# AnnSeidel/genometools

Hardware: AMD Instinct MI355X
Metric: Gbp/s ESA build (suf+lcp+bwt), 3 Gbp DNA, 1/2/4/8 MI355X; bit-exact vs CPU (higher is better)
Workload: dtype u64; 1 GPU; human-like DNA (2% N, 24 seqs, repeats) n=3000000000 seed=43 -suf -lcp -bwt (BASELINE.json configs[2]); parallelism=1 device, pair_suffixes=341032298, tied_suffixes=390540711, refine_rounds=9, maxbranchdepth=8256

## Files before the change

genometools_amd/_lib.py:

```python
import ctypes
import os
import subprocess

HERE = os.path.dirname(os.path.abspath(__file__))
ROOT = os.path.dirname(HERE)
LIB_PATH = os.path.join(HERE, "libgtamd_esa.so")
SOURCES = [os.path.join(HERE, "csrc", f) for f in
           ("esa_prims.hip", "esa_engine.hip", "esa_synth.hip", "esa_encode.hip",
            "esa_pck.hip", "esa_comm.hip")]
HEADERS = [os.path.join(HERE, "csrc", f) for f in ("esa_common.h", "esa_prims.h", "esa_devutil.h", "esa_msd.h", "esa_msd_blocks.h",
                                                     "esa_pck_replay.h")] + \
          [os.path.join(ROOT, "include", h) for h in ("gtamd_esa.h", "gtamd_encode.h", "gtamd_pck.h")]
HIPCC = os.environ.get("HIPCC", "/opt/rocm/bin/hipcc")


def needs_build():
    if not os.path.exists(LIB_PATH):
        return True
    t = os.path.getmtime(LIB_PATH)
    return any(os.path.getmtime(p) > t for p in SOURCES + HEADERS)


def build_library(force=False, verbose=False):
    if not force and not needs_build():
        return LIB_PATH
    cmd = [HIPCC, "--offload-arch=gfx950", "-O3", "-std=c++17", "-fPIC",
           "-shared", "-Wall", "-Wno-unused-function", "-o", LIB_PATH] + SOURCES
    if verbose:
        print(" ".join(cmd))
    subprocess.run(cmd, check=True)
    return LIB_PATH


class EsaStats(ctypes.Structure):
    _fields_ = [("totallength", ctypes.c_uint64),
                ("numberofallsortedsuffixes", ctypes.c_uint64),
                ("longest", ctypes.c_uint64),
                ("largelcpvalues", ctypes.c_uint64),
                ("maxbranchdepth", ctypes.c_uint64),
                ("lcptabsum", ctypes.c_uint64),
                ("prefixlength", ctypes.c_uint32),
                ("refine_rounds", ctypes.c_uint32),
                ("tied_suffixes", ctypes.c_uint64),
                ("pair_suffixes", ctypes.c_uint64),
                ("device_bytes", ctypes.c_uint64),
                ("msd_big_entries", ctypes.c_uint64),
                ("msd_crowded_entries", ctypes.c_uint64),
                ("rank_entries_built", ctypes.c_uint64)]


class EsaTiming(ctypes.Structure):
    _fields_ = [("total_ms", ctypes.c_float),
                ("keygen_ms", ctypes.c_float),
                ("sort_ms", ctypes.c_float),
                ("finalize_ms", ctypes.c_float),
                ("refine_ms", ctypes.c_float),
                ("tie_fix_ms", ctypes.c_float),
                ("scatter_ms", ctypes.c_float),
                ("scatter_launches", ctypes.c_uint32),
                ("scatter_items", ctypes.c_uint64),
                ("comm_ms", ctypes.c_float),
                ("comm_calls", ctypes.c_uint32),
                ("comm_bytes", ctypes.c_uint64),
                ("alloc_ms", ctypes.c_float),
                ("dominant_kernel", ctypes.c_uint32),
                ("scatter_read_items", ctypes.c_uint64),
                ("scatter_written_items", ctypes.c_uint64)]


class EncodeSummary(ctypes.Structure):
    _fields_ = [(name, ctypes.c_uint64) for name in
                ("totallength", "numofsequences", "specialcharacters",
                 "realspecialranges")] + \
               [("specialrangestab", ctypes.c_uint64 * 3)] + \
               [(name, ctypes.c_uint64) for name in
                ("lengthofspecialprefix", "lengthofspecialsuffix", "wildcards",
                 "realwildcardranges")] + \
               [("wildcardrangestab", ctypes.c_uint64 * 3)] + \
               [(name, ctypes.c_uint64) for name in
                ("lengthofwildcardprefix", "lengthofwildcardsuffix",
                 "lengthoflongestnonspecial", "minseqlen", "maxseqlen",
# ... 127 lines not shown
```

genometools_amd/csrc/esa_engine.hip:

```cpp
#include <stdarg.h>
#include <stdlib.h>
#include <chrono>
#include <type_traits>
#include <utility>
#include <vector>
#include "../../include/gtamd_esa.h"
#include "esa_prims.h"
#include "esa_devutil.h"

static thread_local char g_err[1024] = "";
void gtamd_set_error(const char *fmt, ...) {
  va_list ap;
  va_start(ap, fmt);
  vsnprintf(g_err, sizeof g_err, fmt, ap);
  va_end(ap);
}
extern "C" const char *gtamd_esa_last_error(void) { return g_err; }

extern "C" int gtamd_device_count(void) {
  GTAMD_ABI_BEGIN
  int n = 0;
  if (hipGetDeviceCount(&n) != hipSuccess) return 0;
  return n;
  GTAMD_ABI_END(0)
// ... 890 lines not shown
  }
  if (inbucket && (dc != 0 || longk)) {
    u32 letters = K::letters(key);
    if (dc == 0) {
      const u64 sp = sp_window(t, p + K::SYMS);
      letters += sp ? (u32) __ffsll((unsigned long long) sp) - 1u : 64u;
    }
    if (letters < k) {
      atomicAdd(&countspecial[bck_code_long<BITS>(t, key, p, k - 1, sigma)], 1u);
      if (letters >= 1 && letters + 2 <= k) {
        u64 off = 0, pw = sigma;
        for (u32 l = 1; l < letters; l++) { off += pw; pw *= sigma; }
        atomicAdd(&distpfx[off + bck_code_long<BITS>(t, key, p, letters, sigma)], 1u);
      }
    }
  }
}

struct Stats {
  unsigned long long numties;
  unsigned long long lcpsum;
  unsigned long long numlarge;
  unsigned long long longest;
  u32 maxlcp;
  u32 count;
  u32 count2;
  u32 dmax;
  unsigned long long dsum;
  u32 dfallback;
  u32 count3;
  unsigned long long smalldone;
  unsigned long long crowded;
  unsigned long long msum;
};

constexpr int FIN_THREADS = 256;
constexpr int FIN_PER_THREAD = 4;
constexpr int FIN_TILE = FIN_THREADS * FIN_PER_THREAD * 4;

template <int BITS>
__global__ __launch_bounds__(256) void k_tiebits(const u64 *__restrict__ keys,
                                                 u64 N, u64 *__restrict__ tiebits,
                                                 Stats *stats) {
  using K = Key<BITS>;
  __shared__ u32 s_cnt[4];
  const int lane = threadIdx.x & 63, w = threadIdx.x >> 6;
  u32 cnt = 0;
  const u64 ntiles = (N + 4095) / 4096;
  for (u64 tile = blockIdx.x; tile < ntiles; tile += gridDim.x) {
  const u64 wbase = tile * 4096 + (u64) w * 1024;
  u64 k[16];
#pragma unroll
  for (int r = 0; r < 16; r++) {
    const u64 i = wbase + (u64) r * 64 + lane;
    k[r] = i < N ? keys[i] : ~0ull;
  }
  u64 before = (wbase > 0 && wbase < N) ? keys[wbase - 1] : ~k[0];
#pragma unroll
  for (int r = 0; r < 16; r++) {
    const u64 i = wbase + (u64) r * 64 + lane;
    u64 prev = __shfl_up(k[r], 1, 64);
    if (lane == 0) prev = before;
    before = __shfl(k[r], 63, 64);
    const bool tie = i > 0 && i < N && (k[r] >> K::DSHIFT) == (prev >> K::DSHIFT) &&
                     K::dcode(k[r]) == 0;
    const u64 m = __ballot(tie);
// ... 834 lines not shown
      lcp[i + 1] = (u8) (lv < GTAMD_LCPOVERFLOW ? lv : GTAMD_LCPOVERFLOW);
      if (lv >= GTAMD_LCPOVERFLOW) lcpfull[i + 1] = lv;
    }
    if (r & PAIR_SWAP) {
      const u64 x = sa[i], y = sa[i + 1];
      if (x == 0) stats->longest = index_offset + i + 1;
      if (suf != nullptr) { suf[i] = y; suf[i + 1] = x; }
      if (bwt != nullptr) {
        const u8 b0 = bwt[i], b1 = bwt[i + 1];
        bwt[i] = b1;
        bwt[i + 1] = b0;
      }
    }
  }
}

constexpr int RT_TILE = 2048;
constexpr int RT_THREADS = 256;
constexpr int RT_PER = RT_TILE / RT_THREADS;

template <typename P> struct RoundKey {
  static constexpr int KK = sizeof(P) == 8 ? 40 : 32;
  static __device__ __forceinline__ u64 pack(u32 lg, bool open, u64 kk, u32 e) {
    return ((u64) lg << (12 + KK)) | ((u64) open << (11 + KK)) | (kk << 11) | (u64) e;
  }
  static __device__ __forceinline__ bool open(u64 key) { return (key >> (11 + KK)) & 1ull; }
};

template <typename P>
__global__ __launch_bounds__(RT_THREADS) void k_round_tile(
    const u32 *__restrict__ uidx, const P *__restrict__ upos,
    const u32 *__restrict__ ugrp, P *__restrict__ k2, u64 m,
    P *__restrict__ cv, u32 *__restrict__ hv, const u32 *__restrict__ tstart,
    u32 *__restrict__ flagbits, const P *__restrict__ rank, u64 h, u64 n) {
  using RK = RoundKey<P>;
  constexpr bool WIDE = sizeof(P) == 8;
  __shared__ u64 s_key[RT_TILE];
  __shared__ P s_pos[RT_TILE];
  __shared__ u64 s_k2w[WIDE ? RT_TILE : 1];
  __shared__ u16 s_start[RT_TILE + 2];
  __shared__ u32 s_scan[4];
  u32 *s_grp = reinterpret_cast<u32 *>(s_key);
  u32 *s_k2n = s_grp + RT_TILE;
  const int tid = threadIdx.x;
  const u64 tile_first = tstart[blockIdx.x], tile_end = tstart[blockIdx.x + 1];
  for (u64 base = tile_first; base < tile_end; base += RT_TILE) {
  const u32 cnt = (u32) ((tile_end - base) < (u64) RT_TILE ? (tile_end - base) : (u64) RT_TILE);
  const u32 g_first = ugrp[base], g_last = ugrp[base + cnt - 1];
  const bool first_open = base > 0 && ugrp[base - 1] == g_first;
  const bool last_open = base + cnt < m && ugrp[base + cnt] == g_last;
#pragma unroll
  for (int c = 0; c < RT_PER; c++) {
    const u32 e = (u32) c * RT_THREADS + tid;
    P kv = 0;
    if (e < cnt) {
      const P p = upos[base + e];
      s_grp[e] = ugrp[base + e];
      s_pos[e] = p;
      if (rank != nullptr) {
        u64 q = (u64) p + h;
        if (q > n) q = n;
        kv = rank[q];
      } else
        kv = k2[base + e];
    } else {
      s_grp[e] = 0xFFFFFFFFu;
      s_pos[e] = 0;
// ... 11 lines not shown
    gr[c] = s_grp[e0 + c];
    kr[c] = WIDE ? s_k2w[e0 + c] : (u64) s_k2n[e0 + c];
  }
  u32 startflags = 0, nstart = 0;
#pragma unroll
  for (int c = 0; c < RT_PER; c++) {
    const u32 e = e0 + c;
    const bool st = e == 0 || gr[c] != gprev;
    gprev = gr[c];
    startflags |= (u32) st << c;
    nstart += st;
  }
  u32 tot;
  u32 lg = block_scan_excl_sum(nstart, &tot, s_scan);
  u32 nflag = 0;
  int splits = 0;
  u32 openbits = 0;
#pragma unroll
  for (int c = 0; c < RT_PER; c++) {
    const u32 e = e0 + c;
    const bool start = (startflags >> c) & 1u;
    lg += start;
    const u32 g = gr[c];
    const bool open = e < cnt && ((first_open && g == g_first) ||
                                  (last_open && g == g_last));
    const u64 kraw = kr[c];
    const u64 kk = open ? 0ull : kraw;
    splits |= (e < cnt && !open && !start && kraw != kprev);
    kprev = kraw;
    s_key[e] = RK::pack(lg, open, kk, e);
    openbits |= (u32) open << c;
    if (open && rank != nullptr) k2[base + e] = (P) kraw;
    nflag += open;
  }
  if (openbits) {
#pragma unroll
    for (int c = 0; c < RT_PER; c++)
      if ((openbits >> c) & 1u) {
        const u64 slot = base + e0 + c;
        atomicOr(&flagbits[slot >> 5], 1u << (slot & 31));
      }
  }
  const int any_split = __syncthreads_or(splits);
  if (any_split) {
    {
      u32 lgw = lg;
#pragma unroll
      for (int c = RT_PER - 1; c >= 0; c--) {
        const u32 e = e0 + c;
        if ((startflags >> c) & 1u) { s_start[lgw] = (u16) e; lgw--; }
      }
      if (tid == 0) s_start[tot + 1] = (u16) RT_TILE;
    }
    __syncthreads();
    u32 gmax = 0;
    {
      u32 lgw = lg;
#pragma unroll
      for (int c = RT_PER - 1; c >= 0; c--) {
        const u32 e = e0 + c;
        if ((startflags >> c) & 1u) {
          const bool open = RK::open(s_key[e]);
          if (e < cnt && !open) {
            const u32 size = (u32) s_start[lgw + 1] - e;
            gmax = size > gmax ? size : gmax;
          }
// ... 35 lines not shown
            const bool up = (lo & k) == 0;
            const u64 a = s_key[lo], b = s_key[hi];
            if ((a > b) == up) { s_key[lo] = b; s_key[hi] = a; }
          }
          __syncthreads();
        }
      }
    }
  }
  u32 hval[RT_PER], hmax = 0;
#pragma unroll
  for (int c = 0; c < RT_PER; c++) {
    const u32 e = e0 + c;
    const u64 key = s_key[e];
    const bool head = e == 0 || (key >> 11) != (s_key[e - 1] >> 11);
    const u32 v = (head && e < cnt) ? uidx[base + e] : 0u;
    hval[c] = v;
    hmax = v > hmax ? v : hmax;
  }
  u32 carry = block_scan_excl_max(hmax, &tot, s_scan);
#pragma unroll
  for (int c = 0; c < RT_PER; c++) {
    const u32 e = e0 + c;
    carry = hval[c] > carry ? hval[c] : carry;
    if (e < cnt) {
      const u64 key = s_key[e];
      const u32 src = (u32) (key & 2047u);
      if (!RK::open(key)) {
        cv[base + e] = s_pos[src];
        hv[base + e] = carry;
      }
    }
  }
  (void) nflag;
  __syncthreads();
  }
}

constexpr int RT_STRIDE_MIN = 512;
__global__ __launch_bounds__(256) void k_tile_starts(const u32 *__restrict__ ugrp, u64 m,
                                                     u32 ntiles, u32 stride,
                                                     u32 *__restrict__ tstart) {
  const u32 t = blockIdx.x * 256 + threadIdx.x;
  if (t > ntiles) return;
  if (t == ntiles) { tstart[t] = (u32) m; return; }
  const u64 s = (u64) t * stride;
  const u32 g = ugrp[s];
  u64 lo = s > (u64) RT_TILE ? s - RT_TILE : 0, hi = s;
  if (ugrp[lo] == g) {
    tstart[t] = (u32) (lo == 0 ? 0 : s);
    return;
  }
  while (hi - lo > 1) {
    const u64 mid = (lo + hi) >> 1;
    if (ugrp[mid] == g) hi = mid; else lo = mid;
  }
  tstart[t] = (u32) hi;
}

__global__ __launch_bounds__(256) void k_flag_count(const u32 *__restrict__ flagbits, u64 m,
                                                    u32 nblocks, u32 *__restrict__ blkcnt) {
  const u32 b = blockIdx.x * 256 + threadIdx.x;
  if (b >= nblocks) return;
  u32 c = 0;
  for (int w = 0; w < RT_TILE / 32; w++) c += (u32) __popc(flagbits[(u64) b * (RT_TILE / 32) + w]);
  blkcnt[b] = c;
  (void) m;
}

template <typename P>
__global__ __launch_bounds__(RT_THREADS) void k_flag_gather(
    const u32 *__restrict__ flagbits, const u32 *__restrict__ tileoff,
    const u32 *__restrict__ ugrp, const P *__restrict__ k2,
    const P *__restrict__ upos, u64 m, P *__restrict__ fk2, P *__restrict__ fk2_sort,
    u32 *__restrict__ fgrp, P *__restrict__ fpos, u32 *__restrict__ fj,
    u32 *__restrict__ perm) {
  __shared__ u32 s_scan[4];
  const u64 base = (u64) blockIdx.x * RT_TILE + (u64) threadIdx.x * RT_PER;
// ... 21 lines not shown
                                                    const u32 *__restrict__ idx, u64 n,
                                                    u32 *__restrict__ dst) {
  const u64 r = (u64) blockIdx.x * 256 + threadIdx.x;
  if (r < n) dst[r] = src[idx[r]];
}

template <typename P>
__global__ __launch_bounds__(256) void k_flag_heads(
    const u32 *__restrict__ perm, const u32 *__restrict__ fgrp, const P *__restrict__ fk2,
    const P *__restrict__ fpos, const u32 *__restrict__ uidx, const u32 *__restrict__ fj,
    u64 nf, u32 *__restrict__ fhv, P *__restrict__ cvs) {
  const u64 r = (u64) blockIdx.x * 256 + threadIdx.x;
  if (r >= nf) return;
  const u32 a = perm[r];
  bool head = r == 0;
  if (!head) {
    const u32 b = perm[r - 1];
    head = fgrp[a] != fgrp[b] || fk2[a] != fk2[b];
  }
  fhv[r] = head ? uidx[fj[r]] : 0u;
  cvs[r] = fpos[a];
}

template <typename P>
__global__ __launch_bounds__(256) void k_flag_scatter(
    const P *__restrict__ cvs, const u32 *__restrict__ fhv,
    const u32 *__restrict__ fj, u64 nf, P *__restrict__ cv,
    u32 *__restrict__ hv) {
  const u64 r = (u64) blockIdx.x * 256 + threadIdx.x;
  if (r >= nf) return;
  const u32 j = fj[r];
  cv[j] = cvs[r];
  hv[j] = fhv[r];
}

template <typename P>
__global__ __launch_bounds__(256) void k_round_apply(
    const P *__restrict__ cval, const u32 *__restrict__ gnew,
    const u32 *__restrict__ uidx, const u32 *__restrict__ ugrp, u64 m,
    u64 rank_offset, P *__restrict__ sa, P *__restrict__ rank,
    u64 *__restrict__ keep, u32 *__restrict__ blockcnt) {
  __shared__ u32 s_cnt[4];
  const u64 j = (u64) blockIdx.x * 256 + threadIdx.x;
  bool kept = false;
  if (j < m) {
    const P p = cval[j];
    const u32 g = gnew[j], i = uidx[j];
    if (rank != nullptr && g != ugrp[j]) rank[p] = (P) (rank_offset + g);
    const bool head = g == i;
    const bool nexthead = j + 1 == m || gnew[j + 1] == uidx[j + 1];
    const bool resolved = head && nexthead;
    if (resolved) sa[i] = p;
    kept = !resolved;
  }
  const u64 b = __ballot(kept);
  if ((threadIdx.x & 63) == 0) {
    keep[((u64) blockIdx.x * 256 + threadIdx.x) >> 6] = b;
    s_cnt[threadIdx.x >> 6] = (u32) __popcll(b);
  }
  __syncthreads();
  if (threadIdx.x == 0) blockcnt[blockIdx.x] = s_cnt[0] + s_cnt[1] + s_cnt[2] + s_cnt[3];
}

template <typename P>
__global__ __launch_bounds__(256) void k_round_compact(
    const u64 *__restrict__ keep, const u32 *__restrict__ boff,
// ... 259 lines not shown
  for (u64 j = (u64) blockIdx.x * 256 + threadIdx.x; j < m; j += (u64) gridDim.x * 256)
    if (has_letters(t, suf[llv[2 * j] - index_offset], k)) sum += llv[2 * j + 1];
  add_msum(sum, stats);
}

static inline u32 stride_grid(u64 tiles) {
  const u64 cap = 256 * 32;
  return (u32) (tiles < cap ? (tiles ? tiles : 1) : cap);
}

#include "esa_msd.h"

struct Switches {
  int msd = -1;
  bool msd_part_off = false;
  int msd_cbits = -1;
  u32 msd_big_max = MSD_BIG_MAX;
  bool msd_radix = false;
  bool msd_pack = true;
  u32 msd_pack_cap = MD_CAP;
  u32 msd_bin_limit = MD_BIN_LIMIT_DEFAULT;
  bool fused_pass0 = true;
  bool force_wide = false;
  bool no_pairs = false;
  bool no_small_groups = false;
  int apply_early = 2;
  u64 apply_wgs = 0;
  bool apply_wgs_given = false;
  int rank_window_bits = RW_BITS;
  bool rank_all_windows = false;
  bool win_filter_global = false;
  int pair_chunk = 0;
  u32 round_stride = 1536;
  bool debug = false;
};

static Switches read_switches() {
  Switches sw;
  auto flag = [](const char *name, char c) {
    const char *e = getenv(name);
    return e != nullptr && e[0] == c;
  };
  if (const char *e = getenv("GTAMD_MSD")) sw.msd = e[0] == '1';
  sw.msd_part_off = flag("GTAMD_MSD", '0');
  if (const char *e = getenv("GTAMD_MSD_CBITS")) {
    const int v = atoi(e);
    if (v >= 0 && v <= 8) sw.msd_cbits = v;
  }
  if (const char *e = getenv("GTAMD_MSD_BIG_MAX")) {
    const long v = atol(e);
    if (v >= MS_TILE && v <= (long) MSD_BIG_MAX) sw.msd_big_max = (u32) v;
  }
  sw.msd_radix = flag("GTAMD_MSD_RADIX", '1');
  if (const char *e = getenv("GTAMD_MSD_PACK")) sw.msd_pack = atoi(e) != 0;
  if (const char *e = getenv("GTAMD_MSD_PACK_CAP")) {
    const long v = atol(e);
    if (v >= 1024 && v <= (long) MD_CAP) sw.msd_pack_cap = (u32) v;
  }
  if (const char *e = getenv("GTAMD_MSD_BIN_LIMIT")) {
    const long v = atol(e);
    if (v >= 2 && v <= 4096) sw.msd_bin_limit = (u32) v;
  }
  sw.fused_pass0 = !flag("GTAMD_FUSED_PASS0", '0');
  sw.force_wide = flag("GTAMD_FORCE_WIDE", '1');
  sw.no_pairs = flag("GTAMD_NO_PAIRS", '1');
  sw.no_small_groups = flag("GTAMD_NO_SMALL_GROUPS", '1');
  if (const char *e = getenv("GTAMD_APPLY_EARLY")) sw.apply_early = atoi(e);
  if (sw.apply_early < 0 || sw.apply_early > 2) sw.apply_early = 0;
  if (const char *e = getenv("GTAMD_APPLY_WGS")) {
    const long v = atol(e);
    if (v >= 64 && v <= (1 << 22)) sw.apply_wgs = (u64) v;
    sw.apply_wgs_given = true;
  }
  if (const char *e = getenv("GTAMD_RANK_WINDOW_BITS")) {
    const int v = atoi(e);
    if (v >= 2 && v <= RW_BITS) sw.rank_window_bits = v;
  }
  sw.rank_all_windows = flag("GTAMD_RANK_ALL_WINDOWS", '1');
  sw.win_filter_global = flag("GTAMD_WIN_FILTER_LDS", '0');
  if (const char *e = getenv("GTAMD_PAIR_CHUNK")) {
    const int v = atoi(e);
    if (v >= 4 && v <= 1024) sw.pair_chunk = v;
  }
  if (const char *e = getenv("GTAMD_ROUND_STRIDE")) {
    const int v = atoi(e);
    if (v >= RT_STRIDE_MIN && v <= RT_TILE) sw.round_stride = (u32) v;
  }
  sw.debug = getenv("GTAMD_DEBUG") != nullptr;
  return sw;
}

struct DevBuf {
  void *p;
  u64 bytes;
  template <typename T> T *as() const { return reinterpret_cast<T *>(p); }
};

struct gtamd_esa_ctx {
  int device;
  u32 sigma;
  int bits;
  u64 max_n, n, N;
  int readmode;
  hipStream_t st, st2;
  hipEvent_t ev_sorted, ev_emitted, ev_applied;
  DevBuf tb_own, sp_own;
  Text text;
  bool have_text;
  DevBuf k0, k1, v0, v1;
  DevBuf isa_tmp;
  DevBuf rws;
  DevBuf msd;
  DevBuf suf, lcp, bwt;
  DevBuf tiebits, tiebits2;
  DevBuf arena;
  DevBuf arena_p;
  DevBuf xrecv;
  DevBuf winbuf;
  DevBuf lcpfull_buf;
// ... 884 lines not shown
      pcnt = carry + nw + 16;
      poff = pcnt + nw + 16;
      scnt = poff + nw + 16;
      soff = scnt + nw + 16;
      rcnt = soff + nw + 16;
      roff = rcnt + nw + 16;
      scanws = roff + nw + 16;
      pws = scanws + scan_workspace_words(nw) + 64;
    }
  } wd;

  struct PairLists {
    P *pk_a, *pk_b;
    u64 *pv_a, *pv_b;
    u32 *pidx, *pres, *prws, *sidx, *sres, *slcp, *srec;
    u8 *ssize;
    u64 *swp;
    void carve(Bump &a, u64 records, u64 pairs, u64 groups, u64 nw) {
      const u64 pp = (records + 64 + 3) & ~3ull;
      const u64 sp = (groups + 64 + 3) & ~3ull;
      pk_a = a.take<P>(pp); pk_b = a.take<P>(pp);
      pv_a = a.take<u64>(pp); pv_b = a.take<u64>(pp);
      pidx = a.take<u32>(pp); pres = a.take<u32>(pp);
      prws = a.take<u32>(radix_workspace_words(records));
      sidx = a.take<u32>(sp); sres = a.take<u32>(sp); slcp = a.take<u32>(3 * sp);
      srec = a.take<u32>(sp);
      ssize = a.take<u8>(sp);
      swp = a.take<u64>(pairs > 0 ? 2 * nw + 8 : 0);
    }
  } pl;
  const u64 *pair_swp = nullptr;
  int apply_early = 0;
  u64 apply_wgs = 256;
  u32 *lcpfull = nullptr;

  struct Rounds {
    u32 *uidx0, *uidx, *ugrp, *uidx2, *ugrp2;
    P *upos, *upos2;
    P *cvo;
    u32 *hv;
    u64 *keep;
    u32 *koff;
    P *k2;
    u32 *flagbits;
    u32 *tstart;
    P *fk2, *fk2s_a, *fk2s_b, *fpos, *cvs;
    u32 *fgrp, *fj, *perm_a, *perm_b, *gk_a, *gk_b, *fhv;
    P *lk_a, *lk_b;
    u32 *lv_a, *lv_b;
    u32 *rws2, *scanws2;
    u32 *xoff, *xorder, *xqoff, *xmsg, *xbc_q, *xbo_q, *xbc_u, *xbo_u;
    P *xrank, *xans;
    u8 *xdest_q, *xdest_u;
    void carve(Bump &a, u64 mp, u64 tied, u64 items, u32 parts, bool exchange) {
      uidx0 = a.take<u32>(mp); uidx = a.take<u32>(mp); ugrp = a.take<u32>(mp);
      uidx2 = a.take<u32>(mp); ugrp2 = a.take<u32>(mp);
      upos = a.take<P>(mp); upos2 = a.take<P>(mp);
      cvo = a.take<P>(mp);
      hv = a.take<u32>(mp);
      keep = a.take<u64>(mp / 64 + 4);
      koff = a.take<u32>(mp);
      k2 = a.take<P>(mp);
      flagbits = a.take<u32>(mp / 32 + RT_TILE / 32 + 64);
      tstart = a.take<u32>(mp / RT_STRIDE_MIN + 64);
      fk2 = a.take<P>(mp); fk2s_a = a.take<P>(mp); fk2s_b = a.take<P>(mp);
      fpos = a.take<P>(mp); cvs = a.take<P>(mp);
      fgrp = a.take<u32>(mp); fj = a.take<u32>(mp);
      perm_a = a.take<u32>(mp); perm_b = a.take<u32>(mp);
      gk_a = a.take<u32>(mp); gk_b = a.take<u32>(mp);
      fhv = a.take<u32>(mp);
      lk_a = a.take<P>(mp); lk_b = a.take<P>(mp);
      lv_a = a.take<u32>(mp); lv_b = a.take<u32>(mp);
      rws2 = a.take<u32>(radix_workspace_words(tied));
      scanws2 = a.take<u32>(scan_workspace_words(mp > dest_words(parts, items) ? mp : dest_words(parts, items)));
      xoff = xorder = xqoff = xmsg = xbc_q = xbo_q = xbc_u = xbo_u = nullptr;
      xrank = xans = nullptr;
      xdest_q = xdest_u = nullptr;
      if (exchange) {
        xoff = a.take<u32>(items + 64); xorder = a.take<u32>(items + 64);
        xrank = a.take<P>(items + 64); xans = a.take<P>(items + 64);
        xqoff = a.take<u32>(items + 64);
        xmsg = a.take<u32>((items + 64) * (RANKREC + 1));
        xdest_q = a.take<u8>(items + 64); xdest_u = a.take<u8>(items + 64);
        xbc_q = a.take<u32>(dest_words(parts, items)); xbo_q = a.take<u32>(dest_words(parts, items));
        xbc_u = a.take<u32>(dest_words(parts, items)); xbo_u = a.take<u32>(dest_words(parts, items));
      }
    }
  } ar;
  u64 xm = 0;
  u64 xrecv_n = 0;
  u32 *xrecv_msg = nullptr;
  P *xrecv_ans = nullptr;
  P *rank = nullptr;
  P *isa = nullptr;

  struct RankWindows {
    int wb = 0;
// ... 1033 lines not shown
      HIP_TRY(hipGetLastError());
    }
    if (tr.qpre[R] > 0) {
      k_fuse_answers<P><<<(u32) div_up(tr.qpre[R], 256), 256, 0, st>>>(tr, xrecv_msg, isa, xrecv_ans);
      HIP_TRY(hipGetLastError());
    }
    if (m > 0) {
      k_local_lookups<P><<<(u32) div_up(m, 256), 256, 0, st>>>(s.rq, m);
      HIP_TRY(hipGetLastError());
    }
    TRY(comm_alltoallv(c, xrecv_ans, rqc.data(), ar.xans, sq.data(), sizeof(P), "answers"));
    if (ts.qpre[R] > 0) {
      k_k2_scatter<P><<<(u32) div_up(ts.qpre[R], 256), 256, 0, st>>>(ar.xans, ar.xorder, ts.qpre[R], ar.k2);
      HIP_TRY(hipGetLastError());
    }
    return 0;
  }

  int refine_round(RoundState &s) {
    const u64 m = s.m, h = s.h;
    if (!dist && rk.windows && h > rk.h0) {
      HIP_TRY(hipMemsetAsync(&c->d_stats->count2, 0, 4, st));
      k_win_check<P><<<(u32) div_up(m, 256), 256, 0, st>>>(ar.upos, m, h, rk.wb, rk.nwin, rk.w_built,
                                                         rk.w_need, c->d_stats);
      HIP_TRY(hipGetLastError());
      TRY(fetch_stats(c));
      if (c->h_stats->count2 != 0) TRY(build_rank(false));
    }
    const u32 rt_stride = sw.round_stride;
    const u32 g = (u32) div_up(m, 256);
    const u32 ntiles = (u32) div_up(m, rt_stride);
    const u32 nfb = (u32) div_up(m, RT_TILE);
    u32 *tilecnt = ar.koff, *tileoff = ar.koff + nfb + 16;
    HIP_TRY(hipMemsetAsync(ar.flagbits, 0, (u64) nfb * (RT_TILE / 8), st));
    k_tile_starts<<<ntiles / 256 + 1, 256, 0, st>>>(ar.ugrp, m, ntiles, rt_stride, ar.tstart);
    HIP_TRY(hipGetLastError());
    k_round_tile<P><<<ntiles, RT_THREADS, 0, st>>>(
        ar.uidx, ar.upos, ar.ugrp, ar.k2, m, ar.cvo, ar.hv, ar.tstart, ar.flagbits, dist ? nullptr : rank, h, n);
    HIP_TRY(hipGetLastError());
    k_flag_count<<<nfb / 256 + 1, 256, 0, st>>>(ar.flagbits, m, nfb, tilecnt);
    HIP_TRY(hipGetLastError());
    TRY(scan_u32(SCAN_SUM, tilecnt, tileoff, nfb, false, ar.scanws2, st));
    k_total<<<1, 1, 0, st>>>(tileoff, tilecnt, nfb, c->d_stats);
    HIP_TRY(hipGetLastError());
    TRY(fetch_stats(c));
    const u64 nf = c->h_stats->count;
    if (debug)
      fprintf(stderr, "gtamd: part %u round %u: %llu entries in groups across tile borders "
              "(%u tiles, stride %u)\n", c->part, rounds, (unsigned long long) nf, ntiles, rt_stride);
    if (nf > 0) {
      k_flag_gather<P><<<nfb, RT_THREADS, 0, st>>>(ar.flagbits, tileoff, ar.ugrp, ar.k2, ar.upos, m, ar.fk2,
                                                     ar.fk2s_a, ar.fgrp, ar.fpos, ar.fj, ar.perm_a);
      HIP_TRY(hipGetLastError());
      TRY(radix_sort_pairs<P, u32>(ar.fk2s_a, ar.perm_a, ar.fk2s_b, ar.perm_b, nf, ps, pw, pn, ar.rws2, st,
                                   nullptr, nullptr));
      u32 *perm1 = (pn & 1) ? ar.perm_b : ar.perm_a, *permx = (pn & 1) ? ar.perm_a : ar.perm_b;
      const u32 gf = (u32) div_up(nf, 256);
      k_gather_u32<<<gf, 256, 0, st>>>(ar.fgrp, perm1, nf, ar.gk_a);
      HIP_TRY(hipGetLastError());
      TRY(radix_sort_pairs<u32, u32>(ar.gk_a, perm1, ar.gk_b, permx, nf, s.gs, s.gw, s.gn, ar.rws2, st,
                                     nullptr, nullptr));
      const u32 *perm2 = (s.gn & 1) ? permx : perm1;
      k_flag_heads<P><<<gf, 256, 0, st>>>(perm2, ar.fgrp, ar.fk2, ar.fpos, ar.uidx, ar.fj, nf, ar.fhv, ar.cvs);
      HIP_TRY(hipGetLastError());
      TRY(scan_u32(SCAN_MAX, ar.fhv, ar.fhv, nf, true, ar.scanws2, st));
      k_flag_scatter<P><<<gf, 256, 0, st>>>(ar.cvs, ar.fhv, ar.fj, nf, ar.cvo, ar.hv);
      HIP_TRY(hipGetLastError());
    }
    u32 *bcnt = ar.koff, *boffs = ar.koff + g + 16;
    k_round_apply<P><<<g, 256, 0, st>>>(ar.cvo, ar.hv, ar.uidx, ar.ugrp, m, index_offset, sa,
                                        dist ? nullptr : rank, ar.keep, bcnt);
    HIP_TRY(hipGetLastError());
    TRY(scan_u32(SCAN_SUM, bcnt, boffs, g, false, ar.scanws2, st));
    k_round_compact<P><<<g, 256, 0, st>>>(ar.keep, boffs, bcnt, ar.uidx, ar.cvo, ar.hv, m, ar.uidx2,
                                          ar.upos2, ar.ugrp2, c->d_stats);
    HIP_TRY(hipGetLastError());
    TRY(fetch_stats(c));
    s.m = c->h_stats->count;
    s.h *= 2;
    if (dist) {
      s.ru.cval = ar.cvo; s.ru.gnew = ar.hv; s.ru.ugrp = ar.ugrp; s.ru.index_offset = index_offset;
      s.ru.tl = tl; s.ru.isa = isa; s.ru.soff = ar.xoff; s.ru.srank = ar.xrank;
// ... 97 lines not shown
        HIP_TRY(hipGetLastError());
      }
      TRY(fetch_stats(c));
      c->stats.lcptabsum = c->h_stats->msum;
    }
    c->stats.prefixlength = prefixlength;
    c->stats.refine_rounds = rounds;
    c->stats.tied_suffixes = (m0_tied_all ? m0_tied_all : m0) + 2 * npairs + c->h_stats->smalldone;
    c->stats.pair_suffixes = 2 * npairs;
    c->stats.device_bytes = c->alloc_bytes;
    float ms = 0;
    HIP_TRY(hipEventElapsedTime(&ms, c->ev[EV_START], c->ev[EV_DONE])); c->timing.total_ms = ms;
    HIP_TRY(hipEventElapsedTime(&ms, c->ev[EV_START], c->ev[EV_KEYS])); c->timing.keygen_ms = ms;
    HIP_TRY(hipEventElapsedTime(&ms, c->ev[EV_KEYS], c->ev[EV_SORTED])); c->timing.sort_ms = ms;
    HIP_TRY(hipEventElapsedTime(&ms, c->ev[EV_SORTED], c->ev[EV_TIEBITS])); c->timing.finalize_ms = ms;
    HIP_TRY(hipEventElapsedTime(&ms, c->ev[EV_REFINE_BEGIN], c->ev[EV_REFINE_END])); c->timing.refine_ms = ms;
    HIP_TRY(hipEventElapsedTime(&ms, c->ev[EV_REFINE_END], c->ev[EV_DONE])); c->timing.tie_fix_ms = ms;
    float sc = 0;
    for (int i = 0; i < nev; i++) {
      HIP_TRY(hipEventElapsedTime(&ms, c->ev_scatter[2 * i], c->ev_scatter[2 * i + 1]));
      sc += ms;
    }
    if (msd && msd_local > 0) {
      HIP_TRY(hipEventElapsedTime(&sc, c->ev_scatter[0], c->ev_scatter[1]));
      nev = 1;
    }
    c->timing.scatter_ms = sc;
    c->timing.scatter_launches = (u32) nev;
    c->timing.scatter_items = msd ? msd_local : NL;
    c->timing.scatter_read_items = c->timing.scatter_items;
    c->timing.scatter_written_items = msd ? msd_local - c->h_stats->crowded : NL;
    c->stats.msd_crowded_entries = msd ? c->h_stats->crowded : 0;
    c->stats.rank_entries_built = rank_built;
    c->timing.dominant_kernel = msd ? 1u : 0u;
    c->timing.alloc_ms = c->alloc_ms;
    c->want = want;
    c->ran = true;
    return 0;
  }
};

extern "C" int gtamd_esa_run(gtamd_esa_ctx *c, uint32_t want) {
  GTAMD_ABI_BEGIN
  if (c == nullptr) { gtamd_set_error("null context"); return -1; }
  struct AbortOnFailure {
    gtamd_esa_ctx *c;
    bool ok;
    ~AbortOnFailure() {
      if (!ok && c->numparts > 1 && c->comm_abort != nullptr) c->comm_abort(c->comm_abort_user);
    }
  } guard = {c, false};
  if (!c->have_text) { gtamd_set_error("no sequence set"); return -1; }
  if ((want & 15u) == 0) { gtamd_set_error("nothing requested"); return -1; }
  HIP_TRY(hipSetDevice(c->device));
  const Switches sw = read_switches();
  if (sw.debug)
    fprintf(stderr, "gtamd: part %u: switches: msd=%d msd_part_off=%d msd_cbits=%d msd_big_max=%u "
            "msd_radix=%d msd_pack=%d msd_pack_cap=%u msd_bin_limit=%u fused_pass0=%d "
            "force_wide=%d no_pairs=%d no_small_groups=%d apply_early=%d apply_wgs=%llu "
            "apply_wgs_given=%d rank_window_bits=%d rank_all_windows=%d win_filter_global=%d "
            "pair_chunk=%d round_stride=%u debug=%d\n",
            c->part, sw.msd, (int) sw.msd_part_off, sw.msd_cbits, sw.msd_big_max, (int) sw.msd_radix,
            (int) sw.msd_pack, sw.msd_pack_cap, sw.msd_bin_limit, (int) sw.fused_pass0,
            (int) sw.force_wide, (int) sw.no_pairs, (int) sw.no_small_groups, sw.apply_early,
            (unsigned long long) sw.apply_wgs, (int) sw.apply_wgs_given, sw.rank_window_bits,
            (int) sw.rank_all_windows, (int) sw.win_filter_global, sw.pair_chunk, sw.round_stride,
// ... 140 lines not shown
```

include/gtamd_esa.h:

```cpp
#ifndef GTAMD_ESA_H
#define GTAMD_ESA_H

#include <stddef.h>
#include <stdint.h>

#ifdef __cplusplus
extern "C" {
#endif

#define GTAMD_WILDCARD   254u
#define GTAMD_SEPARATOR  255u
#define GTAMD_UNDEFBWT   254u
#define GTAMD_LCPOVERFLOW 255u

#define GTAMD_WANT_SUF 1u
#define GTAMD_WANT_LCP 2u
#define GTAMD_WANT_BWT 4u
#define GTAMD_WANT_BCK 8u

typedef enum {
  GTAMD_TAB_SUF = 0,
  GTAMD_TAB_LCP = 1,
  GTAMD_TAB_BWT = 2,
  GTAMD_TAB_LLV = 3,
  GTAMD_TAB_BCK = 4
} gtamd_table;

typedef struct {
  uint64_t totallength;
  uint64_t numberofallsortedsuffixes;
  uint64_t longest;
  uint64_t largelcpvalues;
  uint64_t maxbranchdepth;
  uint64_t lcptabsum;
  uint32_t prefixlength;
  uint32_t refine_rounds;
  uint64_t tied_suffixes;
  uint64_t pair_suffixes;
  uint64_t device_bytes;
  uint64_t msd_big_entries;
  uint64_t msd_crowded_entries;
  uint64_t rank_entries_built;
} gtamd_esa_stats;

typedef struct {
  float total_ms;
  float keygen_ms;
  float sort_ms;
  float finalize_ms;
  float refine_ms;
  float tie_fix_ms;
  float scatter_ms;
  uint32_t scatter_launches;
  uint64_t scatter_items;
  float comm_ms;
  uint32_t comm_calls;
  uint64_t comm_bytes;
  float alloc_ms;
  uint32_t dominant_kernel;
  uint64_t scatter_read_items;
  uint64_t scatter_written_items;
} gtamd_esa_timing;

typedef struct gtamd_esa_ctx gtamd_esa_ctx;

int gtamd_device_count(void);
const char *gtamd_esa_last_error(void);

uint32_t gtamd_recommended_prefixlength(uint32_t numofchars, uint64_t n);
int gtamd_abi_selftest(uint64_t host_bytes);

gtamd_esa_ctx *gtamd_esa_create(int device, uint64_t max_n,
                                uint32_t numofchars);
void gtamd_esa_destroy(gtamd_esa_ctx *ctx);

// ... 58 lines not shown
```

Before: 26.69 Gbp/s.

## Sort small cross-tile refinement groups in shared memory instead of global radix path

During each refine round, groups that span tile borders are now listed. Each listed group is sized, and groups up to a cap are sorted inside one block using a pivot partition plus a bitonic sort in shared memory, writing cv/hv directly. Only groups above the cap keep going through the global flag-gather and radix path, which can be skipped entirely when there are none. This adds a size-probe kernel and group-sort launches, and it risks slow single-block sorts on large groups near the cap.

New measurement: 26.60 Gbp/s. No clear change (-0.3%).

```diff
diff --git a/genometools_amd/_lib.py b/genometools_amd/_lib.py
--- a/genometools_amd/_lib.py
+++ b/genometools_amd/_lib.py
@@ -46,7 +46,9 @@
                 ("device_bytes", ctypes.c_uint64),
                 ("msd_big_entries", ctypes.c_uint64),
                 ("msd_crowded_entries", ctypes.c_uint64),
-                ("rank_entries_built", ctypes.c_uint64)]
+                ("rank_entries_built", ctypes.c_uint64),
+                ("round_cross_entries", ctypes.c_uint64),
+                ("round_radix_entries", ctypes.c_uint64)]
 
 
 class EsaTiming(ctypes.Structure):
diff --git a/genometools_amd/csrc/esa_engine.hip b/genometools_amd/csrc/esa_engine.hip
--- a/genometools_amd/csrc/esa_engine.hip
+++ b/genometools_amd/csrc/esa_engine.hip
@@ -946,6 +946,7 @@
   unsigned long long smalldone;
   unsigned long long crowded;
   unsigned long long msum;
+  u32 gmax;
 };
 
 constexpr int FIN_THREADS = 256;
@@ -1846,7 +1847,8 @@
     const u32 *__restrict__ uidx, const P *__restrict__ upos,
     const u32 *__restrict__ ugrp, P *__restrict__ k2, u64 m,
     P *__restrict__ cv, u32 *__restrict__ hv, const u32 *__restrict__ tstart,
-    u32 *__restrict__ flagbits, const P *__restrict__ rank, u64 h, u64 n) {
+    u32 *__restrict__ flagbits, const P *__restrict__ rank, u64 h, u64 n,
+    u32 *__restrict__ glist, Stats *stats) {
   using RK = RoundKey<P>;
   constexpr bool WIDE = sizeof(P) == 8;
   __shared__ u64 s_key[RT_TILE];
@@ -1924,6 +1926,14 @@
     openbits |= (u32) open << c;
     if (open && rank != nullptr) k2[base + e] = (P) kraw;
     nflag += open;
+    if (glist != nullptr && open && start && last_open && g == g_last && !(e == 0 && first_open))
+      glist[atomicAdd(&stats->count2, 1u)] = (u32) (base + e);
+  }
+  if (glist != nullptr && __any(openbits != 0)) {
+    u32 w = nflag;
+#pragma unroll
+    for (int d = 32; d >= 1; d >>= 1) w += __shfl_xor(w, d, 64);
+    if ((tid & 63) == 0) atomicAdd(&stats->count, w);
   }
   if (openbits) {
 #pragma unroll
@@ -2025,7 +2035,6 @@
       }
     }
   }
-  (void) nflag;
   __syncthreads();
   }
 }
@@ -2033,10 +2042,14 @@
 constexpr int RT_STRIDE_MIN = 512;
 __global__ __launch_bounds__(256) void k_tile_starts(const u32 *__restrict__ ugrp, u64 m,
                                                      u32 ntiles, u32 stride,
-                                                     u32 *__restrict__ tstart) {
+                                                     u32 *__restrict__ tstart, Stats *stats) {
   const u32 t = blockIdx.x * 256 + threadIdx.x;
   if (t > ntiles) return;
-  if (t == ntiles) { tstart[t] = (u32) m; return; }
+  if (t == ntiles) {
+    tstart[t] = (u32) m;
+    if (stats != nullptr) stats->count = stats->count2 = stats->count3 = stats->gmax = 0u;
+    return;
+  }
   const u64 s = (u64) t * stride;
   const u32 g = ugrp[s];
   u64 lo = s > (u64) RT_TILE ? s - RT_TILE : 0, hi = s;
@@ -2124,6 +2137,127 @@
   const u32 j = fj[r];
   cv[j] = cvs[r];
   hv[j] = fhv[r];
+}
+
+constexpr int RG_CAP = 26624;
+constexpr int RG_CAP_WIDE = 16000;
+constexpr int RG_SMALL = 2048;
+template <typename P> constexpr int rg_cap() { return sizeof(P) == 8 ? RG_CAP_WIDE : RG_CAP; }
+
+__global__ __launch_bounds__(256) void k_group_size(const u32 *__restrict__ ugrp, u64 m,
+                                                    const u32 *__restrict__ glist,
+                                                    u32 *__restrict__ gsize, u32 cap,
+                                                    Stats *stats) {
+  const u32 t = blockIdx.x * 256 + threadIdx.x;
+  if (t >= stats->count2) return;
+  const u64 a = glist[t];
+  const u32 g = ugrp[a];
+  u64 lo = a, hi, step = 1;
+  for (;;) {
+    hi = lo + step;
+    if (hi >= m) { hi = m; break; }
+    if (ugrp[hi] != g) break;
+    lo = hi;
+    step <<= 1;
+  }
+  while (hi - lo > 1) {
+    const u64 mid = (lo + hi) >> 1;
+    if (ugrp[mid] == g) lo = mid; else hi = mid;
+  }
+  const u32 size = (u32) (hi - a);
+  gsize[t] = size;
+  if (size > cap) atomicAdd(&stats->count3, size);
+  else atomicMax(&stats->gmax, size);
+}
+
+template <typename P, int CAPK, int THREADS>
+__global__ __launch_bounds__(THREADS) void k_group_sort(
+    const u32 *__restrict__ uidx, const P *__restrict__ upos, const P *__restrict__ k2,
+    const u32 *__restrict__ glist, const u32 *__restrict__ gsize, P *__restrict__ cv,
+    u32 *__restrict__ hv, u32 *__restrict__ flagbits, u32 cap, int clear) {
+  __shared__ P s_k[CAPK];
+  __shared__ u16 s_i[CAPK];
+  __shared__ u32 s_scan[THREADS / 64];
+  const u32 tid = threadIdx.x;
+  const u64 a = glist[blockIdx.x];
+  const u32 s = gsize[blockIdx.x];
+  if (s > cap || s > (u32) CAPK) return;
+  if (clear) {
+    const u64 z = a + s - 1;
+    const u64 w0 = a >> 5, w1 = z >> 5;
+    const u32 keep0 = ~(~0u << (a & 31)), keep1 = ~(~0u >> (31 - (u32) (z & 31)));
+    if (tid == 0) {
+      if (w0 == w1) atomicAnd(&flagbits[w0], keep0 | keep1);
+      else { atomicAnd(&flagbits[w0], keep0); atomicAnd(&flagbits[w1], keep1); }
+    }
+    for (u64 w = w0 + 1 + tid; w < w1; w += THREADS) flagbits[w] = 0u;
+  }
+  const P pivot = k2[a + (s >> 1)];
+  const u32 c = (s + THREADS - 1) / THREADS;
+  const u32 e0 = tid * c;
+  u32 e1 = e0 + c;
+  if (e1 > s) e1 = s;
+  u32 nl = 0, ne = 0, ng = 0;
+  int unsorted = 0;
+  {
+    P prev = (e0 > 0 && e0 < s) ? k2[a + e0 - 1] : (P) 0;
+    for (u32 e = e0; e < e1; e++) {
+      const P kv = k2[a + e];
+      unsorted |= prev > kv;
+      prev = kv;
+      nl += kv < pivot;
+      ne += kv == pivot;
+      ng += kv > pivot;
+    }
+  }
+  u32 tl, te, tg;
+  u32 pl = block_scan_excl<SCAN_SUM, THREADS>(nl, &tl, s_scan);
+  u32 pe = block_scan_excl<SCAN_SUM, THREADS>(ne, &te, s_scan);
+  u32 pg = block_scan_excl<SCAN_SUM, THREADS>(ng, &tg, s_scan) + tl;
+  const u32 eqhead = uidx[a + tl];
+  for (u32 e = e0; e < e1; e++) {
+    const P kv = k2[a + e];
+    if (kv < pivot) { s_k[pl] = kv; s_i[pl] = (u16) e; pl++; }
+    else if (kv > pivot) { s_k[pg] = kv; s_i[pg] = (u16) e; pg++; }
+    else { cv[a + tl + pe] = upos[a + e]; hv[a + tl + pe] = eqhead; pe++; }
+  }
+  const u32 sc = tl + tg;
+  if (__syncthreads_or(unsorted)) {
+    u32 np2 = 2;
+    while (np2 < sc) np2 <<= 1;
+    const u32 half = np2 >> 1;
+    for (u32 k = 2; k <= np2; k <<= 1) {
+      for (u32 j = k >> 1; j > 0; j >>= 1) {
+        const bool flip = j == (k >> 1);
+        for (u32 idx = tid; idx < half; idx += THREADS) {
+          const u32 lo = ((idx & ~(j - 1)) << 1) | (idx & (j - 1));
+          const u32 hi = flip ? (lo | (k - 1)) - (idx & (j - 1)) : lo + j;
+          if (hi < sc) {
+            const P x = s_k[lo], y = s_k[hi];
+            if (x >= y) {
+              const u16 xi = s_i[lo], yi = s_i[hi];
+              if (x > y || xi > yi) {
+                s_k[lo] = y; s_k[hi] = x;
+                s_i[lo] = yi; s_i[hi] = xi;
+              }
+            }
+          }
+        }
+        __syncthreads();
+      }
+    }
+  }
+  for (u32 q = tid; q < sc; q += THREADS) {
+    const P kv = s_k[q];
+    u32 lo = 0, hi = q;
+    while (lo < hi) {
+      const u32 mid = (lo + hi) >> 1;
+      if (s_k[mid] < kv) lo = mid + 1; else hi = mid;
+    }
+    const u32 skip = q < tl ? 0u : te;
+    cv[a + q + skip] = upos[a + (u32) s_i[q]];
+    hv[a + q + skip] = uidx[a + lo + skip];
+  }
 }
 
 template <typename P>
@@ -2449,6 +2583,7 @@
   bool win_filter_global = false;
   int pair_chunk = 0;
   u32 round_stride = 1536;
+  u32 round_group_max = RG_CAP;
   bool debug = false;
 };
 
@@ -2502,6 +2637,11 @@
   if (const char *e = getenv("GTAMD_ROUND_STRIDE")) {
     const int v = atoi(e);
     if (v >= RT_STRIDE_MIN && v <= RT_TILE) sw.round_stride = (u32) v;
+  }
+  if (const char *e = getenv("GTAMD_ROUND_GROUP_MAX")) {
+    char *end = nullptr;
+    const long v = strtol(e, &end, 10);
+    if (end != e && *end == 0 && v >= 0 && v <= (long) RG_CAP) sw.round_group_max = (u32) v;
   }
   sw.debug = getenv("GTAMD_DEBUG") != nullptr;
   return sw;
@@ -3452,6 +3592,8 @@
   const u64 *pair_swp = nullptr;
   int apply_early = 0;
   u64 apply_wgs = 256;
+  u64 cross_entries = 0;
+  u64 radix_entries = 0;
   u32 *lcpfull = nullptr;
 
   struct Rounds {
@@ -3464,6 +3606,7 @@
     P *k2;
     u32 *flagbits;
     u32 *tstart;
+    u32 *glist, *gsize;
     P *fk2, *fk2s_a, *fk2s_b, *fpos, *cvs;
     u32 *fgrp, *fj, *perm_a, *perm_b, *gk_a, *gk_b, *fhv;
     P *lk_a, *lk_b;
@@ -3483,6 +3626,8 @@
       k2 = a.take<P>(mp);
       flagbits = a.take<u32>(mp / 32 + RT_TILE / 32 + 64);
       tstart = a.take<u32>(mp / RT_STRIDE_MIN + 64);
+      glist = a.take<u32>(mp / RT_STRIDE_MIN + mp / RT_TILE + 64);
+      gsize = a.take<u32>(mp / RT_STRIDE_MIN + mp / RT_TILE + 64);
       fk2 = a.take<P>(mp); fk2s_a = a.take<P>(mp); fk2s_b = a.take<P>(mp);
       fpos = a.take<P>(mp); cvs = a.take<P>(mp);
       fgrp = a.take<u32>(mp); fj = a.take<u32>(mp);
@@ -4582,22 +4727,59 @@
     const u32 ntiles = (u32) div_up(m, rt_stride);
     const u32 nfb = (u32) div_up(m, RT_TILE);
     u32 *tilecnt = ar.koff, *tileoff = ar.koff + nfb + 16;
+    const u32 gcap = sw.round_group_max < (u32) rg_cap<P>() ? sw.round_group_max : (u32) rg_cap<P>();
+    const bool listing = gcap > 0;
     HIP_TRY(hipMemsetAsync(ar.flagbits, 0, (u64) nfb * (RT_TILE / 8), st));
-    k_tile_starts<<<ntiles / 256 + 1, 256, 0, st>>>(ar.ugrp, m, ntiles, rt_stride, ar.tstart);
+    k_tile_starts<<<ntiles / 256 + 1, 256, 0, st>>>(ar.ugrp, m, ntiles, rt_stride, ar.tstart,
+                                                     listing ? c->d_stats : nullptr);
     HIP_TRY(hipGetLastError());
     k_round_tile<P><<<ntiles, RT_THREADS, 0, st>>>(
-        ar.uidx, ar.upos, ar.ugrp, ar.k2, m, ar.cvo, ar.hv, ar.tstart, ar.flagbits, dist ? nullptr : rank, h, n);
+        ar.uidx, ar.upos, ar.ugrp, ar.k2, m, ar.cvo, ar.hv, ar.tstart, ar.flagbits, dist ? nullptr : rank, h, n,
+        listing ? ar.glist : nullptr, c->d_stats);
     HIP_TRY(hipGetLastError());
-    k_flag_count<<<nfb / 256 + 1, 256, 0, st>>>(ar.flagbits, m, nfb, tilecnt);
-    HIP_TRY(hipGetLastError());
-    TRY(scan_u32(SCAN_SUM, tilecnt, tileoff, nfb, false, ar.scanws2, st));
-    k_total<<<1, 1, 0, st>>>(tileoff, tilecnt, nfb, c->d_stats);
-    HIP_TRY(hipGetLastError());
-    TRY(fetch_stats(c));
-    const u64 nf = c->h_stats->count;
+    u64 nf;
+    u64 ncross;
+    if (listing) {
+      const u32 maxgroups = ntiles + nfb + 1;
+      k_group_size<<<maxgroups / 256 + 1, 256, 0, st>>>(ar.ugrp, m, ar.glist, ar.gsize, gcap, c->d_stats);
+      HIP_TRY(hipGetLastError());
+      TRY(fetch_stats(c));
+      ncross = c->h_stats->count;
+      nf = c->h_stats->count3;
+      const u32 ngroups = c->h_stats->count2, gmax = c->h_stats->gmax;
+      if (ngroups > maxgroups) {
+        gtamd_set_error("round %u: %u groups across tile borders listed, %u possible", rounds, ngroups, maxgroups);
+        return -1;
+      }
+      if (gmax > 0) {
+        const int clear = nf > 0;
+        if (gmax <= (u32) RG_SMALL)
+          k_group_sort<P, RG_SMALL, 256><<<ngroups, 256, 0, st>>>(ar.uidx, ar.upos, ar.k2, ar.glist, ar.gsize,
+                                                                  ar.cvo, ar.hv, ar.flagbits, gcap, clear);
+        else
+          k_group_sort<P, rg_cap<P>(), 1024><<<ngroups, 1024, 0, st>>>(ar.uidx, ar.upos, ar.k2, ar.glist, ar.gsize,
+                                                                  ar.cvo, ar.hv, ar.flagbits, gcap, clear);
+        HIP_TRY(hipGetLastError());
+      }
+      if (nf > 0) {
+        k_flag_count<<<nfb / 256 + 1, 256, 0, st>>>(ar.flagbits, m, nfb, tilecnt);
+        HIP_TRY(hipGetLastError());
+        TRY(scan_u32(SCAN_SUM, tilecnt, tileoff, nfb, false, ar.scanws2, st));
+      }
+    } else {
+      k_flag_count<<<nfb / 256 + 1, 256, 0, st>>>(ar.flagbits, m, nfb, tilecnt);
+      HIP_TRY(hipGetLastError());
+      TRY(scan_u32(SCAN_SUM, tilecnt, tileoff, nfb, false, ar.scanws2, st));
+      k_total<<<1, 1, 0, st>>>(tileoff, tilecnt, nfb, c->d_stats);
+      HIP_TRY(hipGetLastError());
+      TRY(fetch_stats(c));
+      ncross = nf = c->h_stats->count;
+    }
+    cross_entries += ncross;
+    radix_entries += nf;
     if (debug)
       fprintf(stderr, "gtamd: part %u round %u: %llu entries in groups across tile borders "
-              "(%u tiles, stride %u)\n", c->part, rounds, (unsigned long long) nf, ntiles, rt_stride);
+              "(%u tiles, stride %u)\n", c->part, rounds, (unsigned long long) ncross, ntiles, rt_stride);
     if (nf > 0) {
       k_flag_gather<P><<<nfb, RT_THREADS, 0, st>>>(ar.flagbits, tileoff, ar.ugrp, ar.k2, ar.upos, m, ar.fk2,
                                                      ar.fk2s_a, ar.fgrp, ar.fpos, ar.fj, ar.perm_a);
@@ -4761,6 +4943,8 @@
     c->timing.scatter_written_items = msd ? msd_local - c->h_stats->crowded : NL;
     c->stats.msd_crowded_entries = msd ? c->h_stats->crowded : 0;
     c->stats.rank_entries_built = rank_built;
+    c->stats.round_cross_entries = cross_entries;
+    c->stats.round_radix_entries = radix_entries;
     c->timing.dominant_kernel = msd ? 1u : 0u;
     c->timing.alloc_ms = c->alloc_ms;
     c->want = want;
diff --git a/include/gtamd_esa.h b/include/gtamd_esa.h
--- a/include/gtamd_esa.h
+++ b/include/gtamd_esa.h
@@ -41,6 +41,8 @@
   uint64_t msd_big_entries;
   uint64_t msd_crowded_entries;
   uint64_t rank_entries_built;
+  uint64_t round_cross_entries;
+  uint64_t round_radix_entries;
 } gtamd_esa_stats;
 
 typedef struct {
```
